# tirtho109/parallel_AMG

Hardware: AMD Instinct MI355X
Metric: V-cycle iters/sec + fine-SpMV HBM GB/s, 3D Poisson 128M dofs at 1/2/4/8 GPU (higher is better)
Workload: dtype f64; 1 GPU; poisson3d 512^3 fp64, SA-AMG V(1,1) weighted-Jacobi, 1 part(s); n=134217728, nnz_fine=937951232, levels=6, max_coarse=1000, parallelism=row-slab partition p1

## Files before the change

### include/pamg.h

```cpp
#ifndef PAMG_H
#define PAMG_H

#include <stdint.h>

#ifdef __cplusplus
extern "C" {
#endif

#define PAMG_OK 0
#define PAMG_E_ARG (-1)
#define PAMG_E_HIP (-2)
#define PAMG_E_RCCL (-3)
#define PAMG_E_OVERFLOW (-4)
#define PAMG_E_SETUP (-5)
#define PAMG_E_STATE (-6)
#define PAMG_E_NOMEM (-7)

typedef struct pamg_ctx pamg_ctx;
typedef struct pamg_plan pamg_plan;
typedef struct pamg_vec pamg_vec;
typedef struct pamg_mat pamg_mat;
typedef struct pamg_hier pamg_hier;
typedef struct pamg_hcsr pamg_hcsr;

// ... 37 lines not shown

int pamg_vec_create(pamg_ctx* ctx, int64_t n_own, int64_t n_ghost, pamg_vec** out);
int pamg_vec_destroy(pamg_vec* v);
int pamg_vec_size(const pamg_vec* v, int64_t* n_own, int64_t* n_ghost);
int pamg_vec_upload(pamg_ctx* ctx, pamg_vec* v, const double* own);
int pamg_vec_download(pamg_ctx* ctx, const pamg_vec* v, double* own);
int pamg_vec_download_ghosts(pamg_ctx* ctx, const pamg_vec* v, double* ghost);
int pamg_vec_device_ptr(pamg_vec* v, double** dptr);
int pamg_vec_fill(pamg_ctx* ctx, pamg_vec* v, double value);
int pamg_vec_fill_xstar(pamg_ctx* ctx, pamg_vec* v, int64_t i0, uint64_t seed);
int pamg_vec_copy(pamg_ctx* ctx, const pamg_vec* src, pamg_vec* dst);
int pamg_vec_axpby(pamg_ctx* ctx, double a, const pamg_vec* x, double b, pamg_vec* y);
int pamg_vec_dot(pamg_ctx* ctx, const pamg_vec* x, const pamg_vec* y, double* out);
int pamg_vec_nrm2(pamg_ctx* ctx, const pamg_vec* x, double* out);
int pamg_exchange(pamg_ctx* ctx, const pamg_plan* plan, pamg_vec* x);
int pamg_exchange_begin(pamg_ctx* ctx, pamg_plan* plan, pamg_vec* x);
int pamg_exchange_end(pamg_ctx* ctx, pamg_plan* plan, pamg_vec* x);

int pamg_mat_upload(pamg_ctx* ctx, int64_t nrows, int64_t ncols_local, const int64_t* rowptr,
                    const void* col, int col_is_64, const double* val, int index_base,
                    const pamg_plan* col_plan, pamg_mat** out);
int pamg_mat_upload_perm(pamg_ctx* ctx, int64_t nrows, int64_t ncols_local, const int64_t* rowptr,
                         const void* col, int col_is_64, const double* val, int index_base,
                         const pamg_plan* col_plan, const int64_t* row_perm,
                         const int64_t* col_perm, pamg_mat** out);
int pamg_mat_upload_blocked(pamg_ctx* ctx, int64_t nrows, int64_t ncols_local, const int64_t* rowptr,
                            const void* col, int col_is_64, const double* val, int index_base,
                            const pamg_plan* col_plan, int bs, pamg_mat** out);
int pamg_mat_destroy(pamg_mat* A);
int pamg_mat_info(const pamg_mat* A, int64_t* nrows, int64_t* ncols_local, int64_t* nnz);
int pamg_mat_stream_bytes(const pamg_mat* A, int64_t* bytes);
int pamg_mat_layout(const pamg_mat* A, int set, int out[10]);
int pamg_mat_ell_window(const pamg_mat* A, int out[16]);

int pamg_mat_set_block_diag(pamg_ctx* ctx, pamg_mat* A, int bs, const double* blocks, const double* inv);
int pamg_mat_block_size(const pamg_mat* A, int* bs);

int pamg_spmv(pamg_ctx* ctx, const pamg_mat* A, pamg_vec* x, pamg_vec* y);
int pamg_residual(pamg_ctx* ctx, const pamg_mat* A, pamg_vec* x, const pamg_vec* b,
                  pamg_vec* r, double* nrm2);
int pamg_jacobi(pamg_ctx* ctx, const pamg_mat* A, pamg_vec* x, const pamg_vec* b,
                pamg_vec* tmp, double omega, int nsweeps);
int pamg_jacobi_residual(pamg_ctx* ctx, const pamg_mat* A, pamg_vec* x, const pamg_vec* b,
                         pamg_vec* t, pamg_vec* r, double omega, int* fused);
int pamg_chebyshev_coeffs(double lmax, double ratio, int degree, double* c1, double* c2);
int pamg_chebyshev(pamg_ctx* ctx, const pamg_mat* A, pamg_vec* x, const pamg_vec* b, pamg_vec* tmp1,
                   pamg_vec* tmp2, double lmax, double ratio, int degree);
int pamg_estimate_lmax(pamg_ctx* ctx, const pamg_mat* A, pamg_vec* v, pamg_vec* y, int steps,
                       int all_parts, double* lam);

int pamg_block_jacobi(pamg_ctx* ctx, const pamg_mat* A, pamg_vec* x, const pamg_vec* b, pamg_vec* tmp,
                      double omega, int nsweeps);
int pamg_block_chebyshev(pamg_ctx* ctx, const pamg_mat* A, pamg_vec* x, const pamg_vec* b, pamg_vec* tmp1,
                         pamg_vec* tmp2, double lmax, double ratio, int degree);
int pamg_estimate_lmax_block(pamg_ctx* ctx, const pamg_mat* A, pamg_vec* v, pamg_vec* y, int steps,
                             int all_parts, double* lam);

int pamg_hier_create(pamg_ctx* ctx, int nlevels, pamg_mat* const* A, pamg_mat* const* P,
                     pamg_mat* const* R, const double* omega, int64_t n_coarse,
                     const double* ainv_colmajor, int rep_level, const int64_t* rep_offsets,
                     pamg_hier** out);
int pamg_hier_destroy(pamg_hier* H);
int pamg_hier_set_graph(pamg_hier* H, int enable);
int pamg_hier_set_sweeps(pamg_hier* H, int nu1, int nu2);
int pamg_hier_set_omega(pamg_hier* H, const double* omega);
#define PAMG_SMOOTHER_JACOBI 0
// ... 67 lines not shown
```

### parallel_amg_amd/_lib.py

```python
from __future__ import annotations

import contextlib
import ctypes as C
import os

_HERE = os.path.dirname(os.path.abspath(__file__))
LIB_PATH = os.environ.get("PAMG_LIB") or os.path.join(_HERE, "libpamg.so")

PAMG_OK = 0
ERRORS = {-1: "PAMG_E_ARG", -2: "PAMG_E_HIP", -3: "PAMG_E_RCCL", -4: "PAMG_E_OVERFLOW",
          -5: "PAMG_E_SETUP", -6: "PAMG_E_STATE", -7: "PAMG_E_NOMEM"}


class PamgError(RuntimeError):
    def __init__(self, code, fn, msg):
        super().__init__(f"{fn} -> {ERRORS.get(code, code)}: {msg}")
        self.code = code


vp = C.c_void_p
i32, i64, dbl = C.c_int, C.c_int64, C.c_double
pvp = C.POINTER(C.c_void_p)
pi64 = C.POINTER(C.c_int64)
pdbl = C.POINTER(C.c_double)
# ... 21 lines not shown
    "pamg_comm_init_local": [vp, vp, i32],
    "pamg_world_spmv": [vp, vp, vp, vp],
    "pamg_world_exchange": [vp, vp, vp],
    "pamg_world_dot": [vp, vp, vp, pdbl],
    "pamg_world_vcycle": [vp, vp, vp, vp, i32, vp],
    "pamg_world_pcg": [vp, vp, vp, vp, dbl, i32, C.POINTER(C.c_int), vp],
    "pamg_plan_create": [vp, i64, i64, i32, vp, vp, vp, vp, pvp],
    "pamg_plan_set_tag": [vp, i64],
    "pamg_plan_destroy": [vp],
    "pamg_vec_create": [vp, i64, i64, pvp],
    "pamg_vec_destroy": [vp],
    "pamg_vec_size": [vp, pi64, pi64],
    "pamg_vec_upload": [vp, vp, vp],
    "pamg_vec_download": [vp, vp, vp],
    "pamg_vec_download_ghosts": [vp, vp, vp],
    "pamg_vec_device_ptr": [vp, pvp],
    "pamg_vec_fill": [vp, vp, dbl],
    "pamg_vec_fill_xstar": [vp, vp, i64, C.c_uint64],
    "pamg_vec_copy": [vp, vp, vp],
    "pamg_vec_axpby": [vp, dbl, vp, dbl, vp],
    "pamg_vec_dot": [vp, vp, vp, pdbl],
    "pamg_vec_nrm2": [vp, vp, pdbl],
    "pamg_exchange": [vp, vp, vp],
    "pamg_exchange_begin": [vp, vp, vp],
    "pamg_exchange_end": [vp, vp, vp],
    "pamg_mat_upload": [vp, i64, i64, vp, vp, i32, vp, i32, vp, pvp],
    "pamg_mat_upload_perm": [vp, i64, i64, vp, vp, i32, vp, i32, vp, vp, vp, pvp],
    "pamg_mat_upload_blocked": [vp, i64, i64, vp, vp, i32, vp, i32, vp, i32, pvp],
    "pamg_mat_destroy": [vp],
    "pamg_mat_info": [vp, pi64, pi64, pi64],
    "pamg_mat_stream_bytes": [vp, pi64],
    "pamg_mat_layout": [vp, i32, C.POINTER(C.c_int)],
    "pamg_mat_ell_window": [vp, C.POINTER(C.c_int)],
    "pamg_mat_set_block_diag": [vp, vp, i32, vp, vp],
    "pamg_mat_block_size": [vp, C.POINTER(C.c_int)],
    "pamg_spmv": [vp, vp, vp, vp],
    "pamg_residual": [vp, vp, vp, vp, vp, pdbl],
    "pamg_jacobi": [vp, vp, vp, vp, vp, dbl, i32],
    "pamg_jacobi_residual": [vp, vp, vp, vp, vp, vp, dbl, pi32],
    "pamg_chebyshev_coeffs": [dbl, dbl, i32, vp, vp],
    "pamg_chebyshev": [vp, vp, vp, vp, vp, vp, dbl, dbl, i32],
    "pamg_estimate_lmax": [vp, vp, vp, vp, i32, i32, vp],
    "pamg_block_jacobi": [vp, vp, vp, vp, vp, dbl, i32],
    "pamg_block_chebyshev": [vp, vp, vp, vp, vp, vp, dbl, dbl, i32],
    "pamg_estimate_lmax_block": [vp, vp, vp, vp, i32, i32, vp],
    "pamg_hier_set_omega": [vp, vp],
    "pamg_hier_create": [vp, i32, vp, vp, vp, vp, i64, vp, i32, vp, pvp],
    "pamg_hier_destroy": [vp],
    "pamg_hier_set_graph": [vp, i32],
    "pamg_hier_set_sweeps": [vp, i32, i32],
    "pamg_hier_set_smoother": [vp, i32, vp, dbl],
    "pamg_hier_set_perm": [vp, i64, vp],
    "pamg_hier_graph_state": [vp, C.POINTER(C.c_int), C.POINTER(C.c_int), C.POINTER(C.c_int)],
    "pamg_vcycle": [vp, vp, vp, vp, i32, vp],
    "pamg_vcycle_async": [vp, vp, vp, vp, i32],
    "pamg_pcg": [vp, vp, vp, vp, dbl, i32, C.POINTER(C.c_int), vp],
    "pamg_pcg_resident": [vp, vp, vp, vp, dbl, i32, i32, C.POINTER(C.c_int), vp, C.POINTER(C.c_int)],
    "pamg_pcg_rr_threshold": [dbl, pdbl],
    "pamg_hier_profile": [vp, i32],
    "pamg_hier_profile_read": [vp, vp],
    "pamg_bench_rowop": [vp, vp, i32, vp, vp, vp, dbl, i32, pdbl],
    "pamg_hier_bench_chain": [vp, vp, vp, i32, pdbl],
    "pamg_set_option": [C.c_char_p, i64],
    "pamg_get_option": [C.c_char_p, pi64],
    "pamg_hcsr_create": [i64, i64, i64, pvp],
    "pamg_hcsr_destroy": [vp],
# ... 57 lines not shown
            continue
        info = _DlInfo()
        if addr and dladdr(addr, C.byref(info)) and info.dli_fname:
            out[key] = os.path.realpath(info.dli_fname.decode())
    return out


def call(name, *args):
    L = lib()
    rc = getattr(L, name)(*args)
    if rc != PAMG_OK:
        msg = L.pamg_last_error().decode(errors="replace")
        raise PamgError(rc, name, msg)
    return rc


@contextlib.contextmanager
def option(key: str, value: int):
    old = C.c_int64()
    call("pamg_get_option", key.encode(), C.byref(old))
    call("pamg_set_option", key.encode(), int(value))
    try:
        yield
    finally:
        call("pamg_set_option", key.encode(), old.value)


def layout_of(M, part_set: int = 0) -> dict:
    out = (C.c_int * 10)()
    call("pamg_mat_layout", M.handle, part_set, out)
    win = (C.c_int * 16)()
    if part_set == 0:
        call("pamg_mat_ell_window", M.handle, win)
    return {"ell_xwin": bool(win[0]), "ell_xwin_groups": int(win[1]), "ell_gather_groups": int(win[2]),
            "ell_xwin_max_window": int(win[3]), "ell_xwin_noncontig_groups": int(win[4]),
            "ell_xwin_max_pairs": int(win[5]), "ell_xwin_max_chunks": int(win[6]),
            "ell_xwin_census": {"groups": int(win[7]), "full_groups": int(win[13]), "window_mean": int(win[8]),
                                "window_p95": int(win[9]), "runs_mean": int(win[10]), "runs_max": int(win[11]),
                                "pairs_mean": int(win[12])},
            "c24": bool(out[0]), "vd": bool(out[1]), "rl8": bool(out[2]), "cd": int(out[3]),
            "cd_offsets": int(out[4]), "tm": bool(out[5]), "tm_rs": int(out[6]),
            "tile_nnz": int(out[7]), "tiles": int(out[8]), "anchored": bool(out[9] & 1), "per_tile": bool(out[9] & 2),
            "x_stage": bool(out[9] & 4), "sym": bool(out[9] & 8), "sym_rows": 2 if out[9] & 16 else 1,
            "jr_fused": bool(out[9] & 32), "tm_vd": bool(out[9] & 64), "sym_vd": bool(out[9] & 128),
            "ell": bool(out[9] & 512), "pnc": bool(out[9] & 1024),
            "rpat": bool(out[9] & 2048), "pnc_compact": bool(out[9] & 4096),
            "ell_pair": bool(out[9] & 8192), "pnc_tiled": bool(out[9] & 16384),
            "bsr": bool(out[9] & 32768)}


def last_error() -> str:
    return lib().pamg_last_error().decode(errors="replace")


def ptr(a):
    return C.c_void_p(a.ctypes.data) if a is not None and a.size else None
```

### parallel_amg_amd/csrc/kernels.hip

```cpp

#include "pamg_device.h"
#include "div_rn.h"

namespace pamg {
namespace {

__device__ __forceinline__ int wave_incl_scan(int v) {
    const int lane = threadIdx.x & 63, rl = lane & 15;
    int t;
    t = __builtin_amdgcn_mov_dpp(v, 0x111, 0xf, 0xf, false);
    if (rl >= 1) v += t;
    t = __builtin_amdgcn_mov_dpp(v, 0x112, 0xf, 0xf, false);
    if (rl >= 2) v += t;
    t = __builtin_amdgcn_mov_dpp(v, 0x114, 0xf, 0xf, false);
    if (rl >= 4) v += t;
    t = __builtin_amdgcn_mov_dpp(v, 0x118, 0xf, 0xf, false);
    if (rl >= 8) v += t;
    t = __builtin_amdgcn_mov_dpp(v, 0x142, 0xf, 0xf, false);
    if (lane & 16) v += t;
    t = __builtin_amdgcn_mov_dpp(v, 0x143, 0xf, 0xf, false);
    if (lane >= 32) v += t;
    return v;
}

// ... 1500 lines not shown
        for (int e = 0; e < 4; ++e) {
            of[e] = lo[(cq >> (8 * e)) & 255u];
            vv[e] = lv[(vq >> (8 * e)) & 255u];
        }
#pragma unroll
        for (int e = 0; e < 4; ++e) xv[e] = x[4 * q + e < L ? base + of[e] : base];
#pragma unroll
        for (int e = 0; e < 4; ++e) {
            const bool ok = 4 * q + e < L;
            const double p = vv[e] * xv[e];
            const double t = s + p;
            s = ok ? t : s;
            if constexpr (kDiagOp<OP>) dg = ok && of[e] == 0 ? vv[e] : dg;
        }
    }
    double out;
    if constexpr (OP == OP_SPMV) {
        out = s;
    } else if constexpr (OP == OP_RESID) {
        out = pb - s;
    } else if constexpr (OP == OP_JACOBI) {
        const double u = pb - s;
        const double v = omega * u;
        const double w = v / dg;
        out = px + w;
    } else if constexpr (OP == OP_CHEB) {
        out = cheb_step(pb - s, px, pxo, dg, c1, omega);
    } else {
        out = py + s;
    }
    if (in) y[i] = out;
}

template <bool WIN>
__device__ __forceinline__ void ellw_dword(uint32_t cq, int q, int L, int lane, int row,
                                           const double* __restrict__ lv, const uint16_t* __restrict__ lof,
                                           const double* __restrict__ lx, const int* __restrict__ lo,
                                           const double* __restrict__ x, double& s) {
    int of[4];
    double vv[4], xv[4];
#pragma unroll
    for (int e = 0; e < 4; ++e) {
        const uint32_t p = (cq >> (8 * e)) & 255u;
        vv[e] = lv[p];
        if constexpr (WIN) of[e] = (int)lof[p] - 64 + lane;
        else of[e] = lo[p];
    }
#pragma unroll
    for (int e = 0; e < 4; ++e) {
        if constexpr (WIN) xv[e] = lx[4 * q + e < L ? of[e] : lane];
        else xv[e] = x[4 * q + e < L ? row + of[e] : row];
    }
#pragma unroll
    for (int e = 0; e < 4; ++e) {
        const bool ok = 4 * q + e < L;
        const double p = vv[e] * xv[e];
        const double t = s + p;
        s = ok ? t : s;
    }
}

constexpr int kEllwPre = 12;
__device__ __forceinline__ void ellw_load(uint32_t (&cq)[kEllwPre], const uint32_t* __restrict__ cw, int first, int nq,
                                          int q0) {
#pragma unroll
    for (int e = 0; e < kEllwPre; ++e) cq[e] = cw[nq > 0 ? first + min(q0 + e, nq - 1) * kEllW : 0];
}

template <int OP>
__global__ __launch_bounds__(kEllGroup) void k_rows_ellw(int nrows, const int4* __restrict__ gslices,
                                                         const int2* __restrict__ smeta, const uint32_t* __restrict__ cw,
                                                         const uint8_t* __restrict__ len, const uint8_t* __restrict__ dpos,
                                                         const int4* __restrict__ gmeta, const int* __restrict__ otab,
                                                         const double* __restrict__ vtab, const int4* __restrict__ wmeta, const int2* __restrict__ chunks,
                                                         const uint16_t* __restrict__ lofs, int win, int gather_all,
                                                         int ngroups, const double* __restrict__ x,
                                                         const double* __restrict__ b, double* __restrict__ y,
                                                         double omega, double c1 = 0.0,
                                                         const double* __restrict__ xold = nullptr) {
    extern __shared__ double ellw_lds[];
    double* lx = ellw_lds;
    double* lv = ellw_lds + win;
    uint16_t* lof = reinterpret_cast<uint16_t*>(lv + 256);
    const int per = (ngroups + 7) / 8;
    const int g = (blockIdx.x & 7) * per + (blockIdx.x >> 3);
    if (g >= ngroups) return;
    const int tid = threadIdx.x, lane = tid & 63;
    const int w = __builtin_amdgcn_readfirstlane(tid >> 6);
    const int4 gm = gmeta[g], wm = wmeta[g], gs = gslices[g];
    const int np = gm.y;
    const bool windowed = wm.y > 0 && !gather_all;
    const double vtv = vtab[gm.x + (tid < np ? tid : 0)];
    const uint32_t* __restrict__ l32 = reinterpret_cast<const uint32_t*>(lofs + wm.z);
    const uint32_t la = l32[windowed && tid < 2 * np ? tid : 0], lb = l32[windowed && tid + 256 < 2 * np ? tid + 256 : 0];
    const int2 cmv = chunks[wm.x + (w + 4 * lane < wm.y ? w + 4 * lane : 0)];
    const int slice = w == 0 ? gs.x : w == 1 ? gs.y : w == 2 ? gs.z : gs.w;
    const int i = slice * kEllW + lane;
    const bool in = slice >= 0 && i < nrows;
    const int ic = in ? i : 0;
    const int L = in ? (int)len[ic] : 0;
    const int2 sm = smeta[slice >= 0 ? slice : 0];
    const int nq = slice >= 0 ? (sm.y + 3) >> 2 : 0;
    const uint32_t* __restrict__ cp = cw + sm.x + lane;
    double pb = 0.0, px = 0.0, py = 0.0, pxo = 0.0;
    if constexpr (OP == OP_RESID || kDiagOp<OP>) pb = b[ic];
    if constexpr (kDiagOp<OP>) px = x[ic];
    if constexpr (OP == OP_PROLONG) py = y[ic];
    if constexpr (OP == OP_CHEB) pxo = xold ? xold[ic] : 0.0;
    uint32_t dkw = 0u;
    int dk = 255;
    if constexpr (kDiagOp<OP>) {
        dk = in ? (int)dpos[ic] : 255;
        dkw = cw[dk != 255 ? sm.x + lane + (dk >> 2) * kEllW : 0];
    }
    double s = 0.0;
    if (windowed) {
        uint32_t cq[kEllwPre];
        ellw_load(cq, cw, sm.x + lane, nq, 0);
        for (int k = 0; w + 4 * k < wm.y; ++k) {
            const int col = __builtin_amdgcn_readlane(cmv.x, k), sc = __builtin_amdgcn_readlane(cmv.y, k);
            if (lane < (sc >> 16))
                __builtin_amdgcn_global_load_lds(
                    (const __attribute__((address_space(1))) void*)(x + col + 2 * lane),
                    (__attribute__((address_space(3))) void*)(lx + (sc & 0xffff)), 16, 0, 0);
        }
        if (tid < np) lv[tid] = vtv;
        if (tid < 2 * np) reinterpret_cast<uint32_t*>(lof)[tid] = la;
        if (tid + 256 < 2 * np) reinterpret_cast<uint32_t*>(lof)[tid + 256] = lb;
        __syncthreads();
        for (int q0 = 0; q0 < nq; q0 += kEllwPre) {
            if (q0 > 0) ellw_load(cq, cw, sm.x + lane, nq, q0);
#pragma unroll
            for (int e = 0; e < kEllwPre; ++e)
                if (q0 + e < nq)
                    ellw_dword<true>(cq[e], q0 + e, L, lane, ic, lv, lof + w * np, lx, nullptr, x, s);
        }
    } else {
        int* lo = reinterpret_cast<int*>(lx);
        const int otv = otab[gm.x + (tid < np ? tid : 0)];
        if (tid < np) {
            lo[tid] = otv;
            lv[tid] = vtv;
        }
        __syncthreads();
        uint32_t c4 = nq > 0 ? cp[0] : 0u;
        for (int q = 0; q < nq; ++q) {
            const uint32_t cq = c4;
            if (q + 1 < nq) c4 = cp[(q + 1) * kEllW];
            ellw_dword<false>(cq, q, L, lane, ic, lv, nullptr, nullptr, lo, x, s);
        }
    }
    double out;
    if constexpr (OP == OP_SPMV) {
        out = s;
    } else if constexpr (OP == OP_RESID) {
        out = pb - s;
    } else if constexpr (OP == OP_JACOBI) {
        const double u = pb - s;
        const double v = omega * u;
        const double dg = dk != 255 ? lv[(dkw >> (8 * (dk & 3))) & 255u] : 0.0;
        const double wq = v / dg;
        out = px + wq;
    } else if constexpr (OP == OP_CHEB) {
        const double dg = dk != 255 ? lv[(dkw >> (8 * (dk & 3))) & 255u] : 0.0;
        out = cheb_step(pb - s, px, pxo, dg, c1, omega);
    } else {
        out = py + s;
    }
    if (in) y[i] = out;
}

template <int OP, int U>
__global__ __launch_bounds__(kEllGroup) void k_rows_rpat(int nrows, const int* __restrict__ gorder,
                                                         const int* __restrict__ anc, const uint8_t* __restrict__ pid,
                                                         const int2* __restrict__ pmeta, int npat,
                                                         const uint32_t* __restrict__ pent, int nent,
                                                         const double* __restrict__ vtab, int nval, int ngroups,
                                                         const double* __restrict__ x, const double* __restrict__ b,
                                                         double* __restrict__ y, double omega) {
    __shared__ uint32_t le[kRpatEnt];
    __shared__ int2 lm[kRpatMax];
// ... 893 lines not shown
    }
}

template <int OP>
void launch_rpat(const pamg_mat& A, const double* x, const double* b, double* y, double omega, hipStream_t s) {
    const RpatSet& R = A.rpat;
    const int grid = (int)((R.ngroups + 7) / 8 * 8);
    auto go = [&](auto kern) {
        kern<<<grid, kEllGroup, 0, s>>>((int)A.nrows, R.d_gorder, R.d_anc, R.d_pid, R.d_pmeta, R.npat, R.d_pent, R.nent,
                                        R.d_vtab, R.nval, (int)R.ngroups, x, b, y, omega);
    };
    go(k_rows_rpat<OP, 8>);
}

template <int OP, int FUSE>
void launch_bsr(const pamg_mat& A, const double* x, const double* b, double* y, double omega, hipStream_t s, Cheb ch);

template <int OP>
void launch_rows_op(const pamg_mat& A, const TileSet& ts, const double* x, const double* b,
                    double* y, double omega, hipStream_t s, Cheb ch = Cheb{}) {
    if (ts.bsr) launch_bsr<OP, 0>(A, x, b, y, omega, s, ch);
    if (ts.sym) launch_sym<OP>(A, x, b, y, omega, s, ch);
    if (ts.ell) {
        const EllSet& E = A.ell;
        const int grid = (int)((E.ngroups + 7) / 8 * 8);
        auto go = [&](auto kern) {
            kern<<<grid, kEllGroup, 0, s>>>((int)A.nrows, E.d_gorder, E.d_anc, E.d_smeta, E.d_ci, E.d_vi, E.d_len,
                                            E.d_gmeta, E.d_otab, E.d_vtab, (int)E.ngroups, x, b, y, omega, ch.c1,
                                            ch.xold);
        };
        if (E.win) {
            const int win = std::max(E.max_window, 128);
            const size_t lds = sizeof(double) * (size_t)(win + 256) + sizeof(uint16_t) * 4 * 256;
            k_rows_ellw<OP><<<grid, kEllGroup, lds, s>>>(
                (int)A.nrows, E.d_gslices, E.d_smeta, E.d_ci, E.d_len, E.d_dpos, E.d_gmeta, E.d_otab, E.d_vtab, E.d_wmeta,
                E.d_chunks, E.d_lof, win, (reinterpret_cast<uintptr_t>(x) & 15) != 0 ? 1 : 0, (int)E.ngroups, x, b, y,
                omega, ch.c1, ch.xold);
        } else if (E.d_anc) {
            if (E.paired) go(k_rows_ell<OP, true, true>);
            else go(k_rows_ell<OP, true, false>);
        } else {
            if (E.paired) go(k_rows_ell<OP, false, true>);
            else go(k_rows_ell<OP, false, false>);
        }
    }
    if constexpr (OP != OP_CHEB) {
        if (ts.pnc) launch_pnc<OP>(A, x, b, y, omega, s);
        if (ts.rpat) launch_rpat<OP>(A, x, b, y, omega, s);
    }
    if (ts.n_short > 0) {
        if (ts.tile_nnz == 1024) launch_tile<OP, 1024>(A, ts, x, b, y, omega, s, ch);
        else if (ts.tile_nnz == 4096) launch_tile<OP, 4096>(A, ts, x, b, y, omega, s, ch);
        else launch_tile<OP, 2048>(A, ts, x, b, y, omega, s, ch);
    }
    if (ts.n_long > 0)
        k_rows_long<OP><<<ts.n_long, kBlock, 0, s>>>(ts.d_long, A.d_rowptr, A.d_col, A.d_val, x,
                                                     b, y, omega, ch.c1, ch.xold);
}


__global__ __launch_bounds__(kBlock) void k_pcg_alpha(int np, const double* __restrict__ partials, PcgScalars* S) {
    if (S->done) return;
    __shared__ double lds[kBlock / 64];
    double v = 0.0;
    for (int i = threadIdx.x; i < np; i += kBlock) v += partials[i];
    const double s = block_sum(v, lds);
    if (threadIdx.x == 0) {
        S->pq = s;
        S->alpha = S->rz / s;
    }
// ... 361 lines not shown
```

### parallel_amg_amd/csrc/matrix.hip

```cpp
#include <algorithm>
#include <array>
#include <atomic>
#include <chrono>
#include <cstdint>
#include <cstdio>
#include <cstdlib>
#include <cstring>
#include <functional>
#include <iterator>
#include <memory>
#include <mutex>
#include <new>
#include <thread>
#include <utility>
#include <vector>

#include "pamg_device.h"
#include "pamg_host.h"

namespace {

int host_threads() {
    static const int n = [] {
        const char* e = std::getenv("OMP_NUM_THREADS");
// ... 954 lines not shown
        std::sort(ws.begin(), ws.end());
        E.p95_window = ws[(ws.size() - 1) * 95 / 100];
        E.mean_window = (int)(win_slots / E.win_groups);
        E.mean_runs = (int)(win_runs / E.win_groups);
        E.mean_pairs = (int)(win_pairs / E.win_groups);
    }
    std::vector<int4> gmeta(ng), wmeta(ng), gsl(ng);
    int64_t on = 0, cn = 0, ln = 0;
    for (int64_t g = 0; g < ng; ++g) {
        const int np = (int)goff[g].size();
        gmeta[g] = make_int4((int)on, np, (int)on, np);
        wmeta[g] = make_int4((int)cn, (int)gchunk[g].size(), (int)ln, gwin[g]);
        gsl[g] = make_int4(grp[g][0], grp[g][1], grp[g][2], grp[g][3]);
        on += np;
        cn += (int64_t)gchunk[g].size();
        ln += (int64_t)glof[g].size();
    }
    if (ln >= INT32_MAX || cn >= INT32_MAX) {
        E = pamg::EllSet{};
        return PAMG_OK;
    }
    std::vector<int> otab(on + 1, 0);
    std::vector<double> vtab(on + 1, 0.0);
    std::vector<int2> chunks(cn + 1, make_int2(0, 0));
    std::vector<uint16_t> lof(ln + 2, (uint16_t)0);
    par_for(ng, [&](int64_t a, int64_t b) {
        for (int64_t g = a; g < b; ++g) {
            std::copy(goff[g].begin(), goff[g].end(), otab.begin() + gmeta[g].x);
            for (size_t e = 0; e < gval[g].size(); ++e) std::memcpy(&vtab[gmeta[g].x + e], &gval[g][e], 8);
            std::copy(gchunk[g].begin(), gchunk[g].end(), chunks.begin() + wmeta[g].x);
            std::copy(glof[g].begin(), glof[g].end(), lof.begin() + wmeta[g].z);
        }
    });
    pamg_ctx* ctx = A->ctx;
    E.nslices = ns;
    E.ngroups = ng;
    E.words = words;
    E.otab_n = on;
    E.vtab_n = on;
    E.paired = true;
    E.win = true;
    E.nchunks = cn;
    E.lof_n = ln;
    CHECK(dalloc(&E.d_smeta, ns));
    CHECK(dalloc(&E.d_ci, words + 1));
    CHECK(dalloc(&E.d_len, n + kVecPad));
    CHECK(dalloc(&E.d_gmeta, ng));
    CHECK(dalloc(&E.d_otab, on + 1));
    CHECK(dalloc(&E.d_vtab, on + 1));
    CHECK(dalloc(&E.d_gslices, ng));
    CHECK(dalloc(&E.d_wmeta, ng));
    CHECK(dalloc(&E.d_chunks, cn + 1));
    CHECK(dalloc(&E.d_lof, ln + 2));
    CHECK(dalloc(&E.d_dpos, n + kVecPad));
    CHECK(h2d(ctx, E.d_dpos, dpos.data(), dpos.size()));
    CHECK(h2d(ctx, E.d_smeta, smeta.data(), sizeof(int2) * ns));
    CHECK(h2d(ctx, E.d_ci, cw.data(), sizeof(uint32_t) * (words + 1)));
    CHECK(h2d(ctx, E.d_len, len.data(), len.size()));
    CHECK(h2d(ctx, E.d_gmeta, gmeta.data(), sizeof(int4) * ng));
    CHECK(h2d(ctx, E.d_otab, otab.data(), sizeof(int) * (on + 1)));
    CHECK(h2d(ctx, E.d_vtab, vtab.data(), sizeof(double) * (on + 1)));
    CHECK(h2d(ctx, E.d_gslices, gsl.data(), sizeof(int4) * ng));
    CHECK(h2d(ctx, E.d_wmeta, wmeta.data(), sizeof(int4) * ng));
    CHECK(h2d(ctx, E.d_chunks, chunks.data(), sizeof(int2) * (cn + 1)));
    CHECK(h2d(ctx, E.d_lof, lof.data(), sizeof(uint16_t) * (ln + 2)));
    A->interior.ell = true;
    return PAMG_OK;
}

int build_ell(pamg_mat* A, const PtrVec& rp, const IdxVec& ci, const double* val,
              bool anchored, const std::vector<int>& inner) {
    using pamg::kEllGroup;
    using pamg::kEllSkip;
    using pamg::kEllW;
    const int64_t n = A->nrows;
    std::vector<char> in_set;
    if ((int64_t)inner.size() != n) {
        in_set.assign(n, 0);
        for (int i : inner) in_set[i] = 1;
    }
    auto member = [&](int64_t i) { return in_set.empty() || in_set[i]; };
    auto base_of = [&](int64_t i) -> int { return anchored ? (rp[i + 1] > rp[i] ? ci[rp[i]] : 0) : (int)i; };
    const int64_t ns = (n + kEllW - 1) / kEllW, ng = (n + kEllGroup - 1) / kEllGroup;
    std::vector<int> slen(ns, 0);
    std::atomic<bool> ok{true};
    par_for(ns, [&](int64_t a, int64_t b) {
        for (int64_t q = a; q < b; ++q) {
            int m = 0;
            for (int64_t i = q * kEllW; i < std::min(n, (q + 1) * kEllW); ++i)
                if (member(i)) m = std::max<int>(m, (int)(rp[i + 1] - rp[i]));
// ... 163 lines not shown
    CHECK(h2d(ctx, E.d_len, len.data(), len.size()));
    CHECK(h2d(ctx, E.d_gmeta, gmeta.data(), sizeof(int4) * ng));
    CHECK(h2d(ctx, E.d_otab, otab.data(), sizeof(int) * (on + 1)));
    CHECK(h2d(ctx, E.d_vtab, vtab.data(), sizeof(double) * (vn + 1)));
    if (anchored) {
        std::vector<int> anc(n + kVecPad, 0);
        par_for(n, [&](int64_t a, int64_t b) {
            for (int64_t i = a; i < b; ++i) anc[i] = base_of(i);
        });
        CHECK(dalloc(&E.d_anc, n + kVecPad));
        CHECK(h2d(ctx, E.d_anc, anc.data(), sizeof(int) * anc.size()));
        CHECK(blocked_group_order(ctx, anc, ng, A->plan ? A->plan->n_own : A->ncols, &E.d_gorder));
    }
    A->interior.ell = true;
    return PAMG_OK;
}

int ell_try(Upload& u) {
    pamg_mat* A = u.A;
    const int64_t nrows = A->nrows, n_own_cols = u.n_own_cols;
    if (pamg::options().ell && !A->interior.sym && !A->interior.rpat && n_own_cols >= nrows && nrows > 0 &&
        (int64_t)u.inner.size() * 4 >= (int64_t)nrows * 3 && nrows >= pamg::options().ell_min_rows &&
        (n_own_cols == nrows || pamg::options().ell_restrict)) {
        CHECK(build_ell(A, u.rp, u.ci, u.val, n_own_cols != nrows, u.inner));
        if (A->interior.ell) u.inner.clear();
        u.tr.mark("ell");
    }
    return PAMG_OK;
}

int64_t ell_bytes(const pamg_mat* A) {
    if (!A->interior.ell) return 0;
    const int64_t nrows = A->nrows;
    return (A->ell.paired ? 4 : 8) * A->ell.words + nrows + 8 * A->ell.nslices + 16 * A->ell.ngroups + 4 * A->ell.otab_n +
           8 * A->ell.vtab_n + (A->ell.d_anc ? 4 * nrows : 0) +
           (A->ell.win ? 32 * A->ell.ngroups + 8 * A->ell.nchunks + 2 * A->ell.lof_n + nrows : 0);
}

void ell_report(const pamg_mat* A, const pamg::TileSet& t, int out[10]) {
    if (!t.ell) return;
    out[8] = (int)A->ell.ngroups;
    out[9] |= 512 | (A->ell.paired ? 8192 : 0);
}

void ell_window(const pamg_mat* A, int out[16]) {
    const pamg::EllSet& E = A->ell;
    const bool w = A->interior.ell && E.win;
    out[0] = w ? 1 : 0;
    out[1] = w ? E.win_groups : 0;
    out[2] = w ? E.gather_groups : 0;
    out[3] = w ? E.max_window : 0;
    out[4] = w ? E.noncontig_groups : 0;
    out[5] = w ? E.max_pairs : 0;
    out[6] = w ? E.max_chunks : 0;
    out[7] = w ? (int)E.ngroups : 0;
    out[8] = w ? E.mean_window : 0;
    out[9] = w ? E.p95_window : 0;
    out[10] = w ? E.mean_runs : 0;
    out[11] = w ? E.max_runs : 0;
    out[12] = w ? E.mean_pairs : 0;
    out[13] = w ? E.full_groups : 0;
    out[14] = out[15] = 0;
}

void ell_free(pamg::EllSet& E) {
    dfree(E.d_gorder);
    dfree(E.d_smeta);
    dfree(E.d_ci);
    dfree(E.d_vi);
    dfree(E.d_len);
    dfree(E.d_gmeta);
    dfree(E.d_otab);
    dfree(E.d_vtab);
    dfree(E.d_anc);
    dfree(E.d_gslices);
    dfree(E.d_wmeta);
    dfree(E.d_chunks);
    dfree(E.d_lof);
    dfree(E.d_dpos);
    E = pamg::EllSet{};
}


int build_pnc(pamg_mat* A, const PtrVec& rp, const IdxVec& ci, const double* val,
              const std::array<int64_t, 4>& grid, const std::vector<int>& inner) {
    using pamg::kPncMaxLen;
    using pamg::kPncSkip;
    const int64_t n = A->nrows;
    std::vector<char> in_set;
    if ((int64_t)inner.size() != n) {
        in_set.assign(n, 0);
        for (int i : inner) in_set[i] = 1;
    }
    auto member = [&](int64_t i) { return in_set.empty() || in_set[i]; };
    const int64_t nx = grid[1], ny = grid[2], nz = grid[3], M = nx * ny;
    if (n != nx * ny * nz || n <= 0 || M % 256 != 0) return PAMG_OK;
    std::vector<int> anc(n + kVecPad, 0);
    std::atomic<bool> ok{true};
// ... 1321 lines not shown

int pamg_mat_info(const pamg_mat* A, int64_t* nrows, int64_t* ncols, int64_t* nnz) {
    if (!A) return fail(PAMG_E_ARG, "mat_info: NULL");
    if (nrows) *nrows = A->nrows;
    if (ncols) *ncols = A->ncols;
    if (nnz) *nnz = A->nnz;
    return PAMG_OK;
}

int pamg_mat_stream_bytes(const pamg_mat* A, int64_t* bytes) {
    if (!A || !bytes) return fail(PAMG_E_ARG, "mat_stream_bytes: bad args");
    *bytes = A->stream_bytes;
    return PAMG_OK;
}

int pamg_mat_layout(const pamg_mat* A, int set, int out[10]) {
    if (!A || !out || set < 0 || set > 1) return fail(PAMG_E_ARG, "mat_layout: bad args");
    const pamg::TileSet& t = set == 0 ? A->interior : A->boundary;
    tiles_report(A, t, out);
    ell_report(A, t, out);
    rpat_report(A, t, out);
    pnc_report(A, t, out);
    sym_report(A, t, out);
    bsr_report(A, t, out);
    return PAMG_OK;
}

int pamg_mat_ell_window(const pamg_mat* A, int out[16]) {
    if (!A || !out) return fail(PAMG_E_ARG, "mat_ell_window: bad args");
    ell_window(A, out);
    return PAMG_OK;
}

}
```

### parallel_amg_amd/csrc/pamg_device.h

```cpp
#pragma once

#include <hip/hip_runtime.h>
#include <rccl/rccl.h>

#include <atomic>
#include <cstdint>
#include <array>
#include <mutex>
#include <vector>

#include "pamg_common.h"

namespace pamg {

constexpr int kBlock = 256;
constexpr int kTileRows = 256;

constexpr int kXsMaxClusters = 12;
constexpr int kTmSmallTab = 128;
constexpr int kXsCap = 1088;
constexpr int kXsIoff = 128;
constexpr int kXsGap = 48;
struct XStage {
    int ncl = 0, stride = 0, zix = -1, ncols = 0;
// ... 96 lines not shown
};
constexpr int kEllW = 64;
constexpr int kEllGroup = 256;
constexpr int kEllSkip = 255;
constexpr int kEllWinCap = 7168;
constexpr int kEllWinChunks = 256;
constexpr int kEllLdsPerCu = 160 * 1024;
constexpr int kEllWinKeep = 85;
constexpr int kEllWinMinShare = 50;
constexpr int kEllWinMinRatio100 = 150;
struct EllSet {
    int64_t nslices = 0, ngroups = 0;
    int2* d_smeta = nullptr;
    uint32_t* d_ci = nullptr;
    uint32_t* d_vi = nullptr;
    uint8_t* d_len = nullptr;
    int4* d_gmeta = nullptr;
    int* d_otab = nullptr;
    double* d_vtab = nullptr;
    int* d_anc = nullptr;
    int* d_gorder = nullptr;
    int64_t words = 0, otab_n = 0, vtab_n = 0;
    bool paired = false;
    bool win = false;
    int4* d_gslices = nullptr;
    int4* d_wmeta = nullptr;
    int2* d_chunks = nullptr;
    uint16_t* d_lof = nullptr;
    uint8_t* d_dpos = nullptr;
    int64_t nchunks = 0, lof_n = 0;
    int win_groups = 0, gather_groups = 0, noncontig_groups = 0;
    int max_window = 0, max_pairs = 0, max_chunks = 0;
    int mean_window = 0, p95_window = 0, mean_runs = 0, max_runs = 0, mean_pairs = 0, full_groups = 0;
};

constexpr int kPncPatMax = 1024, kPncValMax = 128, kPncMaxLen = 7;
constexpr int kPncSkip = kPncPatMax - 1;
constexpr int kPncCombMax = 1024;
constexpr int kPncCombSkip = 0xffff;
constexpr int kPncTx = 64, kPncTy = 4;
constexpr bool pnc_tiled(int nx, int ny) { return nx % kPncTx == 0 && ny % kPncTy == 0; }
struct PncSet {
    int nx = 0, ny = 0, nz = 0;
    int* d_anc = nullptr;
    uint2* d_rec = nullptr;
    uint16_t* d_cid = nullptr;
    uint64_t* d_pvals = nullptr;
    uint32_t* d_ptab = nullptr;
    double* d_vtab = nullptr;
    int npat = 0, nval = 0;
    int grid = 0;
};

constexpr int kRpatMax = 255, kRpatEnt = 4096, kRpatMaxLen = 128;
constexpr int kRpatSkip = 255;
struct RpatSet {
    int64_t ngroups = 0;
    int* d_anc = nullptr;
    uint8_t* d_pid = nullptr;
    int2* d_pmeta = nullptr;
    uint32_t* d_pent = nullptr;
    double* d_vtab = nullptr;
    int* d_gorder = nullptr;
    int npat = 0, nent = 0, nval = 0;
};

// ... 165 lines not shown
```

### parallel_amg_amd/csrc/runtime.hip

```cpp
#include <dlfcn.h>

#include <algorithm>
#include <atomic>
#include <chrono>
#include <cmath>
#include <condition_variable>
#include <cstddef>
#include <cstdint>
#include <cstdio>
#include <cstring>
#include <limits>
#include <memory>
#include <mutex>
#include <string>
#include <thread>
#include <utility>
#include <vector>

#include "pamg_device.h"
#include "pamg_host.h"

pamg::Options& pamg::options() {
    static Options o;
    return o;
// ... 2251 lines not shown
    bool pow2;
};
using O = pamg::Options;
const OptionRow kOptionTable[] = {
    {"tile_nnz", &O::tile_nnz, 1024, 4096, true},
    {"tile_order", &O::tile_order, 0, 1, false},
    {"poison_ghosts", &O::poison_ghosts, 0, 1, false},
    {"col24", &O::col24, 0, 1, false},
    {"long_tiles", &O::long_tiles, 0, 1, false},
    {"row_len8", &O::row_len8, 0, 1, false},
    {"value_dict", &O::value_dict, 0, 2, false},
    {"col_dict", &O::col_dict, 0, 1, false},
    {"tile_major", &O::tile_major, 0, 2, false},
    {"col_dict_anchor", &O::col_dict_anchor, 0, 1, false},
    {"col_dict_tile", &O::col_dict_tile, 0, 1, false},
    {"x_stage", &O::x_stage, 0, 1, false},
    {"band_pct", &O::band_pct, 1, 10000, false},
    {"band_pct_restrict", &O::band_pct_restrict, 1, 10000, false},
    {"long_tiles_min", &O::long_tiles_min, 1, 255, false},
    {"tm_tile_dicts", &O::tm_tile_dicts, 0, 1, false},
    {"sym_dia", &O::sym_dia, 0, 1, false},
    {"sym_rows", &O::sym_rows, 1, 2, false},
    {"jr_fuse", &O::jr_fuse, 0, 1, false},
    {"sym_vd", &O::sym_vd, 0, 1, false},
    {"symd_chunks", &O::symd_chunks, 1, 4, true},
    {"sym_zm", &O::sym_zm, 0, 1, false},
    {"tb_xfast", &O::tb_xfast, 0, 1, false},
    {"ell", &O::ell, 0, 1, false},
    {"ell_restrict", &O::ell_restrict, 0, 1, false},
    {"pnc", &O::pnc, 0, 2, false},
    {"rpat", &O::rpat, 0, 1, false},
    {"pnc_compact", &O::pnc_compact, 0, 1, false},
    {"ell_pair", &O::ell_pair, 0, 1, false},
    {"ell_xwin", &O::ell_xwin, 0, 1, false},
    {"ell_xwin_max", &O::ell_xwin_max, 2, pamg::kEllWinCap, false},
    {"ell_yblock", &O::ell_yblock, 0, 65536, false},
    {"ell_min_rows", &O::ell_min_rows, 0, INT32_MAX, false},
    {"zm_chunks", &O::zm_chunks, 0, 4096, false},
    {"chain_store_x", &O::chain_store_x, 0, 1, false},
};

const OptionRow* find_option(const char* key) {
    for (const OptionRow& r : kOptionTable)
        if (std::strcmp(r.key, key) == 0) return &r;
    return nullptr;
}
}

extern "C" {

int pamg_set_option(const char* key, int64_t value) {
    if (!key) return fail(PAMG_E_ARG, "set_option: NULL key");
    const OptionRow* r = find_option(key);
    if (!r || value < r->lo || value > r->hi || (r->pow2 && (value & (value - 1)) != 0))
        return fail(PAMG_E_ARG, "set_option: unknown key or bad value: %s=%lld", key, (long long)value);
    pamg::options().*(r->member) = (int)value;
    return PAMG_OK;
}

int pamg_get_option(const char* key, int64_t* value) {
    if (!key || !value) return fail(PAMG_E_ARG, "get_option: bad args");
    const OptionRow* r = find_option(key);
    if (!r) return fail(PAMG_E_ARG, "get_option: unknown key %s", key);
    *value = pamg::options().*(r->member);
    return PAMG_OK;
}

// ... 88 lines not shown
```

Baseline: 226.0 V-cycles/s.

## Deduplicate ELL slice column patterns into per-slice classes with per-row class ids

```diff
diff --git a/include/pamg.h b/include/pamg.h
--- a/include/pamg.h
+++ b/include/pamg.h
@@ -93,6 +93,7 @@
 int pamg_mat_stream_bytes(const pamg_mat* A, int64_t* bytes);
 int pamg_mat_layout(const pamg_mat* A, int set, int out[10]);
 int pamg_mat_ell_window(const pamg_mat* A, int out[16]);
+int pamg_mat_ell_classes(const pamg_mat* A, int64_t out[8]);
 
 int pamg_mat_set_block_diag(pamg_ctx* ctx, pamg_mat* A, int bs, const double* blocks, const double* inv);
 int pamg_mat_block_size(const pamg_mat* A, int* bs);
diff --git a/parallel_amg_amd/_lib.py b/parallel_amg_amd/_lib.py
--- a/parallel_amg_amd/_lib.py
+++ b/parallel_amg_amd/_lib.py
@@ -77,6 +77,7 @@
     "pamg_mat_stream_bytes": [vp, pi64],
     "pamg_mat_layout": [vp, i32, C.POINTER(C.c_int)],
     "pamg_mat_ell_window": [vp, C.POINTER(C.c_int)],
+    "pamg_mat_ell_classes": [vp, pi64],
     "pamg_mat_set_block_diag": [vp, vp, i32, vp, vp],
     "pamg_mat_block_size": [vp, C.POINTER(C.c_int)],
     "pamg_spmv": [vp, vp, vp, vp],
@@ -200,7 +201,14 @@
     win = (C.c_int * 16)()
     if part_set == 0:
         call("pamg_mat_ell_window", M.handle, win)
-    return {"ell_xwin": bool(win[0]), "ell_xwin_groups": int(win[1]), "ell_gather_groups": int(win[2]),
+    cls = (C.c_int64 * 8)()
+    if part_set == 0:
+        call("pamg_mat_ell_classes", M.handle, cls)
+    return {"ell_class": bool(cls[0]),
+            "ell_class_census": {"slices": int(cls[1]), "classes_mean": round(cls[2] / max(cls[1], 1), 2),
+                                 "classes_max": int(cls[3]), "record_bytes": int(cls[4]), "id_bytes": int(cls[5]),
+                                 "replaced_bytes": int(cls[6])},
+            "ell_xwin": bool(win[0]), "ell_xwin_groups": int(win[1]), "ell_gather_groups": int(win[2]),
             "ell_xwin_max_window": int(win[3]), "ell_xwin_noncontig_groups": int(win[4]),
             "ell_xwin_max_pairs": int(win[5]), "ell_xwin_max_chunks": int(win[6]),
             "ell_xwin_census": {"groups": int(win[7]), "full_groups": int(win[13]), "window_mean": int(win[8]),
diff --git a/parallel_amg_amd/csrc/kernels.hip b/parallel_amg_amd/csrc/kernels.hip
--- a/parallel_amg_amd/csrc/kernels.hip
+++ b/parallel_amg_amd/csrc/kernels.hip
@@ -1556,7 +1556,7 @@
     if (in) y[i] = out;
 }
 
-template <bool WIN>
+template <bool WIN, bool FULL = false>
 __device__ __forceinline__ void ellw_dword(uint32_t cq, int q, int L, int lane, int row,
                                            const double* __restrict__ lv, const uint16_t* __restrict__ lof,
                                            const double* __restrict__ lx, const int* __restrict__ lo,
@@ -1572,12 +1572,12 @@
     }
 #pragma unroll
     for (int e = 0; e < 4; ++e) {
-        if constexpr (WIN) xv[e] = lx[4 * q + e < L ? of[e] : lane];
-        else xv[e] = x[4 * q + e < L ? row + of[e] : row];
+        if constexpr (WIN) xv[e] = lx[FULL || 4 * q + e < L ? of[e] : lane];
+        else xv[e] = x[FULL || 4 * q + e < L ? row + of[e] : row];
     }
 #pragma unroll
     for (int e = 0; e < 4; ++e) {
-        const bool ok = 4 * q + e < L;
+        const bool ok = FULL || 4 * q + e < L;
         const double p = vv[e] * xv[e];
         const double t = s + p;
         s = ok ? t : s;
@@ -1586,14 +1586,15 @@
 
 constexpr int kEllwPre = 12;
 __device__ __forceinline__ void ellw_load(uint32_t (&cq)[kEllwPre], const uint32_t* __restrict__ cw, int first, int nq,
-                                          int q0) {
-#pragma unroll
-    for (int e = 0; e < kEllwPre; ++e) cq[e] = cw[nq > 0 ? first + min(q0 + e, nq - 1) * kEllW : 0];
-}
-
-template <int OP>
+                                          int q0, int stride) {
+#pragma unroll
+    for (int e = 0; e < kEllwPre; ++e) cq[e] = cw[nq > 0 ? first + min(q0 + e, nq - 1) * stride : 0];
+}
+
+template <int OP, bool CLS>
 __global__ __launch_bounds__(kEllGroup) void k_rows_ellw(int nrows, const int4* __restrict__ gslices,
                                                          const int2* __restrict__ smeta, const uint32_t* __restrict__ cw,
+                                                         const uint8_t* __restrict__ cid,
                                                          const uint8_t* __restrict__ len, const uint8_t* __restrict__ dpos,
                                                          const int4* __restrict__ gmeta, const int* __restrict__ otab,
                                                          const double* __restrict__ vtab, const int4* __restrict__ wmeta, const int2* __restrict__ chunks,
@@ -1624,8 +1625,11 @@
     const int ic = in ? i : 0;
     const int L = in ? (int)len[ic] : 0;
     const int2 sm = smeta[slice >= 0 ? slice : 0];
-    const int nq = slice >= 0 ? (sm.y + 3) >> 2 : 0;
-    const uint32_t* __restrict__ cp = cw + sm.x + lane;
+    const int nq = slice >= 0 ? ((CLS ? sm.y & 0xff : sm.y) + 3) >> 2 : 0;
+    const int nfull = CLS && slice >= 0 ? __builtin_amdgcn_readfirstlane(((sm.y >> 8) & 0xff) >> 2) : 0;
+    const int stride = CLS ? sm.y >> 16 : kEllW;
+    const int first = sm.x + (CLS ? (in ? (int)cid[ic] : 0) : lane);
+    const uint32_t* __restrict__ cp = cw + first;
     double pb = 0.0, px = 0.0, py = 0.0, pxo = 0.0;
     if constexpr (OP == OP_RESID || kDiagOp<OP>) pb = b[ic];
     if constexpr (kDiagOp<OP>) px = x[ic];
@@ -1635,12 +1639,12 @@
     int dk = 255;
     if constexpr (kDiagOp<OP>) {
         dk = in ? (int)dpos[ic] : 255;
-        dkw = cw[dk != 255 ? sm.x + lane + (dk >> 2) * kEllW : 0];
+        dkw = cw[dk != 255 ? first + (dk >> 2) * stride : 0];
     }
     double s = 0.0;
     if (windowed) {
         uint32_t cq[kEllwPre];
-        ellw_load(cq, cw, sm.x + lane, nq, 0);
+        ellw_load(cq, cw, first, nq, 0, stride);
         for (int k = 0; w + 4 * k < wm.y; ++k) {
             const int col = __builtin_amdgcn_readlane(cmv.x, k), sc = __builtin_amdgcn_readlane(cmv.y, k);
             if (lane < (sc >> 16))
@@ -1653,10 +1657,12 @@
         if (tid + 256 < 2 * np) reinterpret_cast<uint32_t*>(lof)[tid + 256] = lb;
         __syncthreads();
         for (int q0 = 0; q0 < nq; q0 += kEllwPre) {
-            if (q0 > 0) ellw_load(cq, cw, sm.x + lane, nq, q0);
+            if (q0 > 0) ellw_load(cq, cw, first, nq, q0, stride);
 #pragma unroll
             for (int e = 0; e < kEllwPre; ++e)
-                if (q0 + e < nq)
+                if (CLS && q0 + e < nfull)
+                    ellw_dword<true, true>(cq[e], q0 + e, L, lane, ic, lv, lof + w * np, lx, nullptr, x, s);
+                else if (q0 + e < nq)
                     ellw_dword<true>(cq[e], q0 + e, L, lane, ic, lv, lof + w * np, lx, nullptr, x, s);
         }
     } else {
@@ -1670,7 +1676,7 @@
         uint32_t c4 = nq > 0 ? cp[0] : 0u;
         for (int q = 0; q < nq; ++q) {
             const uint32_t cq = c4;
-            if (q + 1 < nq) c4 = cp[(q + 1) * kEllW];
+            if (q + 1 < nq) c4 = cp[(q + 1) * stride];
             ellw_dword<false>(cq, q, L, lane, ic, lv, nullptr, nullptr, lo, x, s);
         }
     }
@@ -2630,10 +2636,14 @@
         if (E.win) {
             const int win = std::max(E.max_window, 128);
             const size_t lds = sizeof(double) * (size_t)(win + 256) + sizeof(uint16_t) * 4 * 256;
-            k_rows_ellw<OP><<<grid, kEllGroup, lds, s>>>(
-                (int)A.nrows, E.d_gslices, E.d_smeta, E.d_ci, E.d_len, E.d_dpos, E.d_gmeta, E.d_otab, E.d_vtab, E.d_wmeta,
-                E.d_chunks, E.d_lof, win, (reinterpret_cast<uintptr_t>(x) & 15) != 0 ? 1 : 0, (int)E.ngroups, x, b, y,
-                omega, ch.c1, ch.xold);
+            auto gow = [&](auto kern) {
+                kern<<<grid, kEllGroup, lds, s>>>((int)A.nrows, E.d_gslices, E.d_smeta, E.d_ci, E.d_cid, E.d_len, E.d_dpos,
+                                                  E.d_gmeta, E.d_otab, E.d_vtab, E.d_wmeta, E.d_chunks, E.d_lof, win,
+                                                  (reinterpret_cast<uintptr_t>(x) & 15) != 0 ? 1 : 0, (int)E.ngroups, x, b,
+                                                  y, omega, ch.c1, ch.xold);
+            };
+            if (E.cls) gow(k_rows_ellw<OP, true>);
+            else gow(k_rows_ellw<OP, false>);
         } else if (E.d_anc) {
             if (E.paired) go(k_rows_ell<OP, true, true>);
             else go(k_rows_ell<OP, true, false>);
diff --git a/parallel_amg_amd/csrc/matrix.hip b/parallel_amg_amd/csrc/matrix.hip
--- a/parallel_amg_amd/csrc/matrix.hip
+++ b/parallel_amg_amd/csrc/matrix.hip
@@ -1010,6 +1010,67 @@
             std::copy(glof[g].begin(), glof[g].end(), lof.begin() + wmeta[g].z);
         }
     });
+    std::vector<int2> smeta_c;
+    std::vector<uint32_t> ccw;
+    std::vector<uint8_t> cid;
+    if (pamg::options().ell_xwin == 1) {
+        std::vector<int> snc(ns, 0), smin(ns, 0);
+        cid.assign(n + kVecPad, 0);
+        par_for(ns, [&](int64_t a, int64_t b) {
+            int rep[kEllW];
+            for (int64_t q = a; q < b; ++q) {
+                const int nq = (smeta[q].y + 3) / 4;
+                const int64_t r0 = q * kEllW, s0 = smeta[q].x;
+                const int rows = (int)std::min<int64_t>(n - r0, kEllW);
+                int nc = 0;
+                for (int l = 0; l < rows; ++l) {
+                    int c = 0;
+                    for (; c < nc; ++c) {
+                        const int m = rep[c];
+                        bool same = len[r0 + l] == len[r0 + m] && dpos[r0 + l] == dpos[r0 + m];
+                        for (int k = 0; k < nq && same; ++k) same = cw[s0 + (int64_t)k * kEllW + l] == cw[s0 + (int64_t)k * kEllW + m];
+                        if (same) break;
+                    }
+                    if (c == nc) rep[nc++] = l;
+                    cid[r0 + l] = (uint8_t)c;
+                }
+                snc[q] = nc;
+                int lmin = rows == kEllW ? 255 : 0;
+                for (int l = 0; l < rows; ++l) lmin = std::min<int>(lmin, len[r0 + l]);
+                smin[q] = lmin;
+            }
+        });
+        smeta_c.resize(ns);
+        int64_t cwords = 0;
+        for (int64_t q = 0; q < ns; ++q) {
+            smeta_c[q] = make_int2((int)cwords, smeta[q].y | smin[q] << 8 | snc[q] << 16);
+            cwords += (int64_t)snc[q] * ((smeta[q].y + 3) / 4);
+            E.cls_total += snc[q];
+            E.cls_max = std::max(E.cls_max, snc[q]);
+        }
+        if (2 * (4 * cwords + n) <= 4 * words) {
+            E.cls = true;
+            E.cls_words = cwords;
+            ccw.assign(cwords + 1, 0u);
+            par_for(ns, [&](int64_t a, int64_t b) {
+                for (int64_t q = a; q < b; ++q) {
+                    const int nq = (smeta[q].y + 3) / 4, nc = snc[q];
+                    const int64_t r0 = q * kEllW, s0 = smeta[q].x;
+                    const int rows = (int)std::min<int64_t>(n - r0, kEllW);
+                    for (int l = 0; l < rows; ++l)
+                        for (int k = 0; k < nq; ++k)
+                            ccw[smeta_c[q].x + (int64_t)k * nc + cid[r0 + l]] = cw[s0 + (int64_t)k * kEllW + l];
+                }
+            });
+            std::vector<uint32_t>().swap(cw);
+        } else {
+            E.cls_total = 0;
+            E.cls_max = 0;
+        }
+    }
+    const std::vector<int2>& sm_up = E.cls ? smeta_c : smeta;
+    const std::vector<uint32_t>& cw_up = E.cls ? ccw : cw;
+    const int64_t up_words = E.cls ? E.cls_words : words;
     pamg_ctx* ctx = A->ctx;
     E.nslices = ns;
     E.ngroups = ng;
@@ -1021,7 +1082,11 @@
     E.nchunks = cn;
     E.lof_n = ln;
     CHECK(dalloc(&E.d_smeta, ns));
-    CHECK(dalloc(&E.d_ci, words + 1));
+    CHECK(dalloc(&E.d_ci, up_words + 1));
+    if (E.cls) {
+        CHECK(dalloc(&E.d_cid, n + kVecPad));
+        CHECK(h2d(ctx, E.d_cid, cid.data(), cid.size()));
+    }
     CHECK(dalloc(&E.d_len, n + kVecPad));
     CHECK(dalloc(&E.d_gmeta, ng));
     CHECK(dalloc(&E.d_otab, on + 1));
@@ -1032,8 +1097,8 @@
     CHECK(dalloc(&E.d_lof, ln + 2));
     CHECK(dalloc(&E.d_dpos, n + kVecPad));
     CHECK(h2d(ctx, E.d_dpos, dpos.data(), dpos.size()));
-    CHECK(h2d(ctx, E.d_smeta, smeta.data(), sizeof(int2) * ns));
-    CHECK(h2d(ctx, E.d_ci, cw.data(), sizeof(uint32_t) * (words + 1)));
+    CHECK(h2d(ctx, E.d_smeta, sm_up.data(), sizeof(int2) * ns));
+    CHECK(h2d(ctx, E.d_ci, cw_up.data(), sizeof(uint32_t) * (up_words + 1)));
     CHECK(h2d(ctx, E.d_len, len.data(), len.size()));
     CHECK(h2d(ctx, E.d_gmeta, gmeta.data(), sizeof(int4) * ng));
     CHECK(h2d(ctx, E.d_otab, otab.data(), sizeof(int) * (on + 1)));
@@ -1263,7 +1328,8 @@
 int64_t ell_bytes(const pamg_mat* A) {
     if (!A->interior.ell) return 0;
     const int64_t nrows = A->nrows;
-    return (A->ell.paired ? 4 : 8) * A->ell.words + nrows + 8 * A->ell.nslices + 16 * A->ell.ngroups + 4 * A->ell.otab_n +
+    const int64_t index = A->ell.cls ? 4 * A->ell.cls_words + nrows : (A->ell.paired ? 4 : 8) * A->ell.words;
+    return index + nrows + 8 * A->ell.nslices + 16 * A->ell.ngroups + 4 * A->ell.otab_n +
            8 * A->ell.vtab_n + (A->ell.d_anc ? 4 * nrows : 0) +
            (A->ell.win ? 32 * A->ell.ngroups + 8 * A->ell.nchunks + 2 * A->ell.lof_n + nrows : 0);
 }
@@ -1294,7 +1360,21 @@
     out[14] = out[15] = 0;
 }
 
+void ell_classes(const pamg_mat* A, int64_t out[8]) {
+    const pamg::EllSet& E = A->ell;
+    const bool c = A->interior.ell && E.cls;
+    out[0] = c ? 1 : 0;
+    out[1] = c ? E.nslices : 0;
+    out[2] = c ? E.cls_total : 0;
+    out[3] = c ? E.cls_max : 0;
+    out[4] = c ? 4 * E.cls_words : 0;
+    out[5] = c ? A->nrows : 0;
+    out[6] = c ? 4 * E.words : 0;
+    out[7] = 0;
+}
+
 void ell_free(pamg::EllSet& E) {
+    dfree(E.d_cid);
     dfree(E.d_gorder);
     dfree(E.d_smeta);
     dfree(E.d_ci);
@@ -2682,4 +2762,10 @@
     return PAMG_OK;
 }
 
-}
+int pamg_mat_ell_classes(const pamg_mat* A, int64_t out[8]) {
+    if (!A || !out) return fail(PAMG_E_ARG, "mat_ell_classes: bad args");
+    ell_classes(A, out);
+    return PAMG_OK;
+}
+
+}
diff --git a/parallel_amg_amd/csrc/pamg_device.h b/parallel_amg_amd/csrc/pamg_device.h
--- a/parallel_amg_amd/csrc/pamg_device.h
+++ b/parallel_amg_amd/csrc/pamg_device.h
@@ -152,6 +152,11 @@
     int win_groups = 0, gather_groups = 0, noncontig_groups = 0;
     int max_window = 0, max_pairs = 0, max_chunks = 0;
     int mean_window = 0, p95_window = 0, mean_runs = 0, max_runs = 0, mean_pairs = 0, full_groups = 0;
+    bool cls = false;
+    uint8_t* d_cid = nullptr;
+    int64_t cls_words = 0;
+    int cls_max = 0;
+    int64_t cls_total = 0;
 };
 
 constexpr int kPncPatMax = 1024, kPncValMax = 128, kPncMaxLen = 7;
diff --git a/parallel_amg_amd/csrc/runtime.hip b/parallel_amg_amd/csrc/runtime.hip
--- a/parallel_amg_amd/csrc/runtime.hip
+++ b/parallel_amg_amd/csrc/runtime.hip
@@ -2307,7 +2307,7 @@
     {"rpat", &O::rpat, 0, 1, false},
     {"pnc_compact", &O::pnc_compact, 0, 1, false},
     {"ell_pair", &O::ell_pair, 0, 1, false},
-    {"ell_xwin", &O::ell_xwin, 0, 1, false},
+    {"ell_xwin", &O::ell_xwin, 0, 2, false},
     {"ell_xwin_max", &O::ell_xwin_max, 2, pamg::kEllWinCap, false},
     {"ell_yblock", &O::ell_yblock, 0, 65536, false},
     {"ell_min_rows", &O::ell_min_rows, 0, INT32_MAX, false},
```

New measurement: 228.4 V-cycles/s (median of 6 runs). 1.01x the previous value.
